# yukara-ikemiya/world-class

Measured on AMD Instinct MI355X. Metric: analysis+synthesis frames/sec (whole node), 48 kHz 5 ms hop, higher is better.
Workload: dtype f64; 1 GPU; 64 synthetic 48 kHz 10 s utterances per GPU (8 distinct, tiled), 5 ms hop, Harvest->CheapTrick->D4C->Synthesis, inputs resident in HBM when the clock starts (`value`; SURVEY.md section 8(d)'s headline with H2D of x and D2H of all outputs inside the clock is `value_with_transfers`); utterances_per_gpu=64, frames_per_gpu=128064, fs=48000, fft_size=2048, parallelism=utterance-sharded x1 (shard.partition), final RCCL all-gather of F0 + checksums

## Files before the change

world_class_amd/csrc/wc_d4c.hip:

```cpp
#include <cmath>
#include <cstdio>
#include <cstdlib>
#include <cstring>
#include <type_traits>
#include <vector>

#include "wc_device.hpp"
#include "wc_internal.hpp"
#include "wc_frames.hpp"
#include "wc_wavefft.hpp"
#include "wc_hostcopy.hpp"

namespace wc {

constexpr double kSafe = 0.000000000001;
constexpr int kMaxBands = 5;

struct D4cArgs {
	const double *x;
	const UttDesc *utts;
	int n_utt;
	const double *tpos, *f0;
	const unsigned long long *rng_off;
	const uint32_t *rng_table;
	unsigned long long rng_base;
	const double2 *tw;
	double *ap;
	double *ap0;
	double *sgd;
	double *coarse;
	uint32_t *cnt;
	const double *nuttall;
	long long total_frames;
	int fs, fft_size_out, n_ap, window_length;
	int select64;
	double threshold;
	long long sgd_stride;
	int *long_list, *long_cnt;
	const int *uidx;
	int rare_only;
	int *rare_list;
};

template <int N, int T>
__device__ __forceinline__ int d4c_windowed(const double *__restrict__ x, int x_len, int fs, double f0, double pos,
											int type, double ratio, const uint32_t *__restrict__ rng,
											unsigned long long roff, double (&wave)[N / T], double *red, int tid) {
	constexpr int EPT = N / T;
	asm volatile("" : "+v"(tid));
	const int hw = mround(ratio * fs / f0 / 2.0);
	const int wl = 2 * hw + 1;
	const int origin = mround(pos * fs + 0.001);
	const double c1 = 2.0 / ratio / fs;
	double cs0, sn0, csd, snd;
	sincospi(f0 * (c1 * (tid - hw)), &sn0, &cs0);
	sincospi(f0 * (c1 * T), &snd, &csd);
	snd = uniform_d(snd);
	csd = uniform_d(csd);
	auto win = [&](double c) { return type == 1 ? fma(0.5, c, 0.5) : fma(c, fma(0.16, c, 0.5), 0.34); };
	double s1 = 0.0, s2 = 0.0;
	{
		double c = cs0, sn = sn0;
#pragma unroll
		for (int e = 0; e < EPT; ++e) {
			const int i = tid + e * T;
			const bool in = i < wl;
			const double w = in ? win(c) : 0.0;
			const int si = clampi(origin + i - hw, 0, x_len - 1);
			const double noise = randn_at(rng, roff + (in ? i : 0)) * kSafe;
			wave[e] = in ? fma(x[si], w, noise) : 0.0;
			s1 += wave[e];
			s2 += w;
			const double cn = fma(c, csd, -(sn * snd));
// ... 57 lines not shown
	if (NONNEG) {
		static_assert(M + 2 >= T + 2 * (T / 64), "P doubles as the scratch of the cumulative sum");
		for (int i = tid; i < len; i += T) S[i] = mir(i) * fs / N;
		__syncthreads();
		seq_cumsum_nonneg<T>(S, len, const_cast<double *>(P), red, tid);
	} else {
		const int ch = (len + T - 1) / T;
		const int lo = tid * ch, hi = min(len, lo + ch);
		double loc = 0.0;
		for (int i = lo; i < hi; ++i) loc += mir(i) * fs / N;
		double run = block_excl_scan<T>(loc, red, tid);
		for (int i = lo; i < hi; ++i) {
			run = mir(i) * fs / N + run;
			S[i] = run;
		}
		__syncthreads();
	}
	const double origin_axis = -(b - 0.5) * fs / N;
	const double step = (double)fs / N, rstep = 1.0 / step;
	auto seg = [&](int i) -> double { return S[min(max(i, 0), len - 1)]; };
	for (int k = tid; k <= M; k += T) {
		double lo_axis = (double)k / N * fs - width / 2.0;
		double hi_axis = lo_axis + width;
		double lo_v = interp1q_rcp(origin_axis, step, rstep, seg, len, lo_axis);
		double hi_v = interp1q_rcp(origin_axis, step, rstep, seg, len, hi_axis);
		out(k, (hi_v - lo_v) / width);
	}
	__syncthreads();
}

__host__ __device__ __forceinline__ bool d4c2_can(double f0, int fs) {
	const int v = (int)(f0 * 4096 / fs);
	return v + 1 <= 120 && v + 2 <= 122;
}

__global__ void d4c_lt_count_kernel(const double *__restrict__ f0, long long total, int fs, uint32_t *__restrict__ cnt,
									const UttDesc *__restrict__ utts, int n_utt, int *__restrict__ uidx, int *__restrict__ long_cnt,
									int *__restrict__ rare_cnt) {
	long long g = (long long)blockIdx.x * blockDim.x + threadIdx.x;
	if (g >= total) return;
	if (g == 0) { *long_cnt = 0; *rare_cnt = 0; }
	uidx[g] = find_utt(utts, n_utt, g);
	double f = f0[g];
	cnt[g] = (f == 0.0) ? 0u : (uint32_t)(2 * mround(3.0 * fs / fmax(f, 40.0) / 2.0) + 1);
}

template <int N, int T>
__global__ __launch_bounds__(T, T == 512 ? 6 : 1) void d4c_lovetrain_kernel(D4cArgs a) {
	constexpr int M = N / 2;
	constexpr int EPT = N / T;
	__shared__ double2 A[fft_lds_size(M)];
	__shared__ double red[2 * (T / 64) + 2];
	double *Ar = reinterpret_cast<double *>(A);
	int tid = threadIdx.x;
	long long g = xcd_frame(blockIdx.x, a.total_frames);
	if (g >= a.total_frames) return;
	const int bins_out = a.fft_size_out / 2 + 1;
	double *__restrict__ row = a.ap + g * (long long)bins_out;
	const double f0v = a.f0[g];
	double ap0 = 0.0;
	if (f0v != 0.0) {
		const int u = find_utt(a.utts, a.n_utt, g);
		const UttDesc ud = a.utts[u];
		const int fs = a.fs;
		const double f0c = fmax(f0v, 40.0);
		double wave[EPT];
// ... 411 lines not shown
		unsigned int acc = inc - own;
		unsigned int d = 4u * lane, cnt;
		if (acc + h4.x >= need) { cnt = h4.x; }
		else if (acc + h4.x + h4.y >= need) { acc += h4.x; d += 1; cnt = h4.y; }
		else if (acc + h4.x + h4.y + h4.z >= need) { acc += h4.x + h4.y; d += 2; cnt = h4.z; }
		else { acc += h4.x + h4.y + h4.z; d += 3; cnt = h4.w; }
		acc = __shfl(acc, first, 64);
		d = __shfl(d, first, 64);
		in_bucket = __shfl(cnt, first, 64);
		need -= acc;
		pre |= ((unsigned long long)d) << shift;
		if (in_bucket == 1u) break;
	}
	double low = 0.0, eq = 0.0, tot = 0.0;
#pragma unroll
	for (int e = 0; e < KEYS; ++e) {
		if (e < nkeys) {
			const double pw = key[e];
			const unsigned long long hb = ((unsigned long long)__double_as_longlong(pw)) >> shift;
			tot += pw;
			low += (hb < (pre >> shift)) ? pw : 0.0;
			eq += (hb == (pre >> shift)) ? pw : 0.0;
		}
	}
	block_sum3<T>(low, eq, tot, red3, tid);
	if (tid == 0) {
		const double thr = (in_bucket == 1u) ? eq : __longlong_as_double((long long)pre);
		const double part = low + (double)need * thr;
		const double cv = 10 * log10(part / tot);
		a.coarse[g * kMaxBands + bnd] = fmin(0.0, cv + (f0 - 100) / 50.0);
	}
}

__global__ __launch_bounds__(256) void d4c_rows_kernel(D4cArgs a) {
	const long long g = blockIdx.x;
	const double f0v = a.f0[g];
	if (f0v == 0.0 || a.ap0[g] <= a.threshold) return;
	const int n_ap = a.n_ap, fs = a.fs;
	const int bins_out = a.fft_size_out / 2 + 1;
	const double *__restrict__ co = a.coarse + g * kMaxBands;
	double *__restrict__ row = a.ap + g * (long long)bins_out;
	const int na = n_ap + 2;
	auto val = [&](int q) { return q == 0 ? -60.0 : (q == na - 1 ? -kSafe : co[q - 1]); };
	for (int k = threadIdx.x; k < bins_out; k += 256) {
		double f = (double)k * fs / a.fft_size_out;
		int c = 1;
		while (c < na && f >= ((c == na - 1) ? fs / 2.0 : c * 3000.0)) ++c;
		c = min(c, na - 1);
		double x0 = (c - 1) * 3000.0;
		double x1 = (c == na - 1) ? fs / 2.0 : c * 3000.0;
		double s = (f - x0) / (x1 - x0);
		double v = val(c - 1) + s * (val(c) - val(c - 1));
		row[k] = exp(v * 0.11512925464970228);
	}
}


constexpr long long kD4Row = 4160;
constexpr int kD4Lds = 2304;

template <int SLOTS>
__device__ __forceinline__ int d4c2_windowed(int type, const double *__restrict__ x, int x_last, int fs, double f0, double pos, double ratio,
											 const uint32_t *__restrict__ rng, int odd, bool weighted, double (&re)[16],
											 double (&im)[16], double &sumsq, int lane) {
	WC_FRESH(lane);
	const int hw = __builtin_amdgcn_readfirstlane(mround(ratio * fs / f0 / 2.0));
	const int wl = 2 * hw + 1;
	const int base = __builtin_amdgcn_readfirstlane(mround(pos * fs + 0.001)) - hw;
	const double c1 = 2.0 / ratio / fs;
	double ce0, se0, co0, so0, cd, sd;
	wf_sincospi(f0 * (c1 * (2 * lane - hw)), se0, ce0);
	wf_sincospi(f0 * (c1 * (2 * lane + 1 - hw)), so0, co0);
	wf_sincospi(f0 * (c1 * 128.0), sd, cd);
	sd = uniform_d(sd);
	cd = uniform_d(cd);
	const double a0 = type == 1 ? 0.5 : 0.34, a2 = type == 1 ? 0.0 : 0.16;
	auto win = [&](double c) { return fma(c, fma(a2, c, 0.5), a0); };
	auto walk = [&](auto loads_c, auto &&body) {
		constexpr int LOADS = decltype(loads_c)::value;
		double ce = ce0, se = se0, co = co0, so = so0;
#pragma unroll
		for (int qg = 0; qg < SLOTS; qg += 4) {
			if (qg * 128 >= wl) break;
			double xs[8];
			uint32_t ns[8];
			const bool ld = LOADS == 1 || (LOADS == 2 && qg >= 16);
			if (ld) {
// ... 108 lines not shown
		ap0 = p1 / p2;
	}
	const bool gate = !(f0v == 0.0 || ap0 <= a.threshold);
	if (lane == 0) {
		a.ap0[g] = ap0;
		a.cnt[g] = gate ? (uint32_t)(3 * (2 * mround(4.0 * a.fs / fmax(47.0, f0v) / 2.0) + 1)) : 0u;
	}
	if (!gate) {
		const double init_val = 1.0 - kSafe;
		for (int k = lane; k < bins_out; k += 64) row[k] = init_val;
	}
}

struct D4Bins {
	double v[2][16];
	double vM;
};
__device__ __forceinline__ void d4c2_dc_correction(D4Bins &s, double f0, int fs, double *L, int lane) {
	constexpr int N = 4096;
	WC_FRESH(lane);
	const int upper = __builtin_amdgcn_readfirstlane(2 + (int)(f0 * N / fs));
	const double dx = -(double)fs / N, rdx = 1.0 / dx;
	L[2 * lane] = s.v[0][0];
	L[2 * lane + 1] = s.v[1][0];
	wf_fence();
	auto rep = [&](int i) {
		const double axis = (double)i * fs / N;
		return interp1q_rcp(f0, dx, rdx, [&](int b) { return L[min(max(b, 0), 127)]; }, upper + 1, axis);
	};
	if (2 * lane < upper - 1) s.v[0][0] += rep(2 * lane);
	if (2 * lane + 1 < upper - 1) s.v[1][0] += rep(2 * lane + 1);
	wf_fence();
}
template <bool NONNEG>
__device__ __forceinline__ void d4c2_smooth(D4Bins &s, double width, int fs, double *L, int lane) {
	constexpr int N = 4096, M = 2048;
	WC_FRESH(lane);
	const int b = __builtin_amdgcn_readfirstlane((int)(width * N / fs) + 1);
	const int len = M + 2 * b + 1;
	int jg[2][4];
#pragma unroll
	for (int p = 0; p < 2; ++p)
#pragma unroll
		for (int gq = 0; gq < 4; ++gq) jg[p][gq] = 2 * wf_j(lane, p, gq) + p;
#pragma unroll
	for (int p = 0; p < 2; ++p)
#pragma unroll
		for (int gq = 0; gq < 4; ++gq)
#pragma unroll
			for (int q = 0; q < 4; ++q) L[jg[p][gq] + 512 * q + b] = s.v[p][4 * gq + q] * fs / N;
	if (lane == 0) L[M + b] = s.vM * fs / N;
	{
		const int ke = 2 * lane, ko = 2 * lane + 1;
		if (ke >= 1 && ke <= b) {
			L[b - ke] = s.v[0][0] * fs / N;
			L[M + b + ke] = s.v[0][7] * fs / N;
		}
		if (ko <= b) {
			L[b - ko] = s.v[1][0] * fs / N;
			L[M + b + ko] = s.v[1][7] * fs / N;
		}
	}
	wf_fence();
	if (NONNEG) {
		seq_cumsum_nonneg_wave<36>(L, len, lane);
	} else {
		seq_cumsum_signed_wave<36>(L, len, lane);
	}
	const double step = (double)fs / N;
	const double origin_axis = -(b - 0.5) * fs / N;
	const double rstep = 1.0 / step;
	const double rwidth = uniform_d(1.0 / width);
	auto at = [&](int k) {
		const double lo_axis = (double)k / N * fs - width / 2.0, hi_axis = lo_axis + width;
		return (wf_interp1q(origin_axis, step, rstep, L, len, hi_axis) - wf_interp1q(origin_axis, step, rstep, L, len, lo_axis)) * rwidth;
	};
#pragma unroll
	for (int p = 0; p < 2; ++p)
#pragma unroll
		for (int gq = 0; gq < 4; ++gq) {
#pragma unroll
			for (int q = 0; q < 4; ++q) s.v[p][4 * gq + q] = at(jg[p][gq] + 512 * q);
			WF_SCHED_FENCE();
		}
	s.vM = at(M);
	wf_fence();
}

#ifndef WC_D4C2_OCC
#define WC_D4C2_OCC 2
#endif
#ifndef WC_D4C2_MASTER_LDS
#define WC_D4C2_MASTER_LDS 1
#endif
#ifndef WC_D4C2_TRACE
#define WC_D4C2_TRACE 0
#endif
#if WC_D4C2_TRACE
#define D4_STAMP(i) do { if (lane == 0) reinterpret_cast<unsigned long long *>(park + 4128)[i] = __builtin_readcyclecounter(); } while (0)
#else
// ... 184 lines not shown
					for (int q = 0; q < 16; ++q) {
						const int i0 = 2 * ln + 128 * q;
						ar[q] *= pw * (i0 + 1.0);
						ai[q] *= pw * (i0 + 2.0);
					}
				}
				wf_r2c4096_half(ar, ai, nyq2, ng, L, a.tw, lane, odd);
#pragma unroll
				for (int s = 0; s < 16; ++s) acc[s] += fma(re[s], ar[s], im[s] * ai[s]);
				accM += nyq1 * nyq2;
				if (odd == 0 && job == 0) D4_STAMP(3);
			}
		}
#pragma unroll
		for (int s = 0; s < 16; ++s) d4_st(row, 1024 * odd + 64 * s + lane, acc[s]);
		if (odd == 0) cenM = accM;
		if (odd == 0) D4_STAMP(4);
	}
	D4_STAMP(5);
	D4Bins cen, sps;
#pragma unroll
	for (int p = 0; p < 2; ++p)
#pragma unroll
		for (int s = 0; s < 16; ++s) {
			cen.v[p][s] = d4_ld(row, 1024 * p + 64 * s + lane);
			sps.v[p][s] = d4_ld(row, 2048 + 1024 * p + 64 * s + lane);
		}
	cen.vM = cenM;
	sps.vM = spsM;
	D4_STAMP(6);
	d4c2_dc_correction(cen, f0, fs, L, lane);
	d4c2_dc_correction(sps, f0, fs, L, lane);
	D4_STAMP(7);
	d4c2_smooth<true>(sps, f0, fs, L, lane);
	D4_STAMP(8);
#pragma unroll
	for (int p = 0; p < 2; ++p)
#pragma unroll
		for (int s = 0; s < 16; ++s) cen.v[p][s] = cen.v[p][s] / sps.v[p][s];
	cen.vM = cen.vM / sps.vM;
#pragma unroll 1
	for (int it = 0; it < 2; ++it) {
		d4c2_smooth<false>(cen, it ? f0 : f0 / 2.0, fs, L, lane);
		if (it == 0) sps = cen;
	}
	D4_STAMP(9);
#pragma unroll
	for (int p = 0; p < 2; ++p)
#pragma unroll
		for (int gq = 0; gq < 4; ++gq) {
			const int j = 2 * wf_j(lane, p, gq) + p;
#pragma unroll
			for (int q = 0; q < 4; ++q) d4_st(row, j + 512 * q, sps.v[p][4 * gq + q] - cen.v[p][4 * gq + q]);
		}
	if (lane == 0) d4_st(row, M, sps.vM - cen.vM);
	D4_STAMP(10);
}

template <bool LONG>
__global__ __launch_bounds__(64) __attribute__((amdgpu_waves_per_eu(WC_D4C2_OCC, WC_D4C2_OCC))) void d4c2_frames_kernel(D4cArgs a) {
	__shared__ __attribute__((aligned(16))) double L[kD4Lds];
	const int lane = threadIdx.x;
	if constexpr (!LONG) {
		const long long g = xcd_frame(blockIdx.x, a.total_frames);
		if (g >= a.total_frames) return;
		d4c2_frame<false>(a, g, L, lane);
	} else {
		const int n_long = *a.long_cnt;
#pragma unroll 1
		for (int i = blockIdx.x; i < n_long; i += gridDim.x) {
			d4c2_frame<true>(a, a.long_list[1 + i], L, lane);
			wf_fence();
		}
	}
}

// ... 7 lines not shown
#define WC_D4C2_BRACKET_FIRST 0x1p-14
#endif
#ifndef WC_D4C2_BAND_PF
#define WC_D4C2_BAND_PF 0
#endif
__global__ __launch_bounds__(64) __attribute__((amdgpu_waves_per_eu(WC_D4C2_BAND_OCC, WC_D4C2_BAND_OCC))) void d4c2_band_kernel(D4cArgs a) {
	constexpr int N = 4096, M = 2048;
	__shared__ __attribute__((aligned(16))) double L[kWfLds];
	const int lane = threadIdx.x;
	const int n_ap = a.n_ap;
	const long long blk = xcd_frame(blockIdx.x, (long long)gridDim.x);
	const long long g = blk / n_ap;
	const int bnd = (int)(blk % n_ap);
	if (g >= a.total_frames) return;
	const double f0v = a.f0[g];
	if (f0v == 0.0 || a.ap0[g] <= a.threshold) return;
	const double f0 = fmax(47.0, f0v);
	const int fs = a.fs;
	const int wln = a.window_length, hwl = wln / 2;
	const int boundary = mround(N * 8.0 / wln);
	const unsigned int K = (unsigned int)(M + 1 - boundary - 1);
	const int center = (int)(3000.0 * (bnd + 1) * N / fs);
	const double *__restrict__ src = a.sgd + g * a.sgd_stride + (center - hwl);
	const int ng = wln > 512 ? 2 : 1;
	double key[2][16], keyM = 0.0;
	[[maybe_unused]] double pf = 0.0;
#pragma unroll
	for (int odd = 0; odd < 2; ++odd) {
		double re[16], im[16], nyq;
		{
			double sv[16], nv[16];
#pragma unroll
			for (int k = 0; k < 16; ++k) {
				const int i = min(2 * lane + 128 * (k >> 1) + (k & 1), wln - 1);
				sv[k] = src[i];
				nv[k] = a.nuttall[i];
			}
#if WC_D4C2_BAND_PF > 0
			if (odd == 0) {
				const long long b2 = min((long long)blockIdx.x + 8ll * WC_D4C2_BAND_PF, (long long)gridDim.x - 1);
				const long long blk2 = xcd_frame(b2, (long long)gridDim.x);
				const long long g2 = min(blk2 / n_ap, a.total_frames - 1);
				const int center2 = (int)(3000.0 * ((int)(blk2 % n_ap) + 1) * N / fs);
				pf = (a.sgd + g2 * a.sgd_stride + (center2 - hwl))[min(16 * lane, wln - 1)];
			}
#endif
			WF_SCHED_FENCE();
#pragma unroll
			for (int q = 0; q < 16; ++q) {
				re[q] = im[q] = 0.0;
				if (q < 8) {
					const int i0 = 2 * lane + 128 * q;
					re[q] = (i0 < wln) ? sv[2 * q] * nv[2 * q] : 0.0;
					im[q] = (i0 + 1 < wln) ? sv[2 * q + 1] * nv[2 * q + 1] : 0.0;
				}
			}
		}
		if (odd) wf_odd_twist(re, im, a.tw, lane, 8);
		if (ng == 1) wdft16<+1, 1>(re, im);
		else wdft16<+1, 2>(re, im);
		wf_fft1024_dit_rest_p<+1>(re, im, L, a.tw, lane, odd);
		if (odd) wf_r2c_unpack_odd(re, im, a.tw, lane);
		else wf_r2c_unpack(re, im, nyq, a.tw, lane);
#pragma unroll
		for (int s = 0; s < 16; ++s) key[odd][s] = fma(re[s], re[s], im[s] * im[s]);
		if (!odd) keyM = nyq * nyq;
	}
	double mx = (lane == 0) ? keyM : 0.0;
#pragma unroll
// ... 65 lines not shown
	for (int p = 0; p < 2; ++p)
#pragma unroll
		for (int s = 0; s < 16; ++s) {
			tot += key[p][s];
			low += (__double_as_longlong(key[p][s]) <= lo) ? key[p][s] : 0.0;
		}
	if (lane == 0) {
		tot += keyM;
		low += (__double_as_longlong(keyM) <= lo) ? keyM : 0.0;
	}
	low = wave_sum_all(low);
	tot = wave_sum_all(tot);
	if (lane == 0) {
		const double part = low + (double)(K - c_lo) * __longlong_as_double(hi);
		const double cv = 10 * log10(part / tot);
		a.coarse[g * kMaxBands + bnd] = fmin(0.0, cv + (f0 - 100) / 50.0);
	}
#if WC_D4C2_BAND_PF > 0
	asm volatile("" ::"v"(pf));
#endif
}


constexpr long long kD4Row1 = 3136;
constexpr int kD4Lds1 = 2176;
__host__ __device__ __forceinline__ bool d4c1_can(double f0, int fs) {
	const int v = (int)(f0 * 2048 / fs);
	return v + 1 <= 120 && v + 2 <= 122;
}
extern "C" int wc_debug_d4c_wave_takes(int fft_size, double f0, int fs) {
	if (fft_size == 4096) return d4c2_can(f0, fs) ? 1 : 0;
	if (fft_size == 2048) return d4c1_can(f0, fs) ? 1 : 0;
	return -1;
}
struct D4Bins1 {
	double v[16];
	double vM;
};
__device__ __forceinline__ void d4c1_dc_correction(D4Bins1 &s, double f0, int fs, double *L, int lane) {
	constexpr int N = 2048;
	WC_FRESH(lane);
	const int upper = __builtin_amdgcn_readfirstlane(2 + (int)(f0 * N / fs));
	const double dx = -(double)fs / N, rdx = 1.0 / dx;
	L[lane] = s.v[0];
	L[64 + lane] = s.v[8];
	wf_fence();
	auto rep = [&](int i) {
		const double axis = (double)i * fs / N;
		return interp1q_rcp(f0, dx, rdx, [&](int b) { return L[min(max(b, 0), 127)]; }, upper + 1, axis);
	};
	if (lane < upper - 1) s.v[0] += rep(lane);
	if (upper - 1 > 64) {
		if (64 + lane < upper - 1) s.v[8] += rep(64 + lane);
	}
	wf_fence();
}
template <bool NONNEG>
__device__ __forceinline__ void d4c1_smooth(D4Bins1 &s, double width, int fs, double *L, int lane) {
	constexpr int N = 2048, M = 1024;
	WC_FRESH(lane);
	const int b = __builtin_amdgcn_readfirstlane((int)(width * N / fs) + 1);
	const int len = M + 2 * b + 1;
	int jg[4];
#pragma unroll
	for (int gq = 0; gq < 4; ++gq) jg[gq] = wf_bin(lane, gq, 0);
#pragma unroll
	for (int gq = 0; gq < 4; ++gq)
#pragma unroll
		for (int q = 0; q < 4; ++q) L[jg[gq] + 256 * q + b] = s.v[4 * gq + q] * fs / N;
	if (lane == 0) L[M + b] = s.vM * fs / N;
	if (lane >= 1 && lane <= b) {
		L[b - lane] = s.v[0] * fs / N;
		L[M + b + lane] = s.v[7] * fs / N;
	}
	if (64 + lane <= b) {
		L[b - 64 - lane] = s.v[8] * fs / N;
		L[M + b + 64 + lane] = s.v[15] * fs / N;
	}
	wf_fence();
	if (NONNEG) seq_cumsum_nonneg_wave<20>(L, len, lane);
	else seq_cumsum_signed_wave<20>(L, len, lane);
	const double step = (double)fs / N;
	const double origin_axis = -(b - 0.5) * fs / N;
	const double rstep = 1.0 / step;
	const double rwidth = uniform_d(1.0 / width);
	auto at = [&](int k) {
		const double lo_axis = (double)k / N * fs - width / 2.0, hi_axis = lo_axis + width;
		return (wf_interp1q(origin_axis, step, rstep, L, len, hi_axis) - wf_interp1q(origin_axis, step, rstep, L, len, lo_axis)) * rwidth;
	};
#pragma unroll
	for (int gq = 0; gq < 4; ++gq) {
#pragma unroll
		for (int q = 0; q < 4; ++q) s.v[4 * gq + q] = at(jg[gq] + 256 * q);
		WF_SCHED_FENCE();
	}
	s.vM = at(M);
	wf_fence();
}

#ifndef WC_D4C1_LT_OCC
#define WC_D4C1_LT_OCC 3
#endif
#ifndef WC_D4C1_OCC
#define WC_D4C1_OCC 2
#endif
#ifndef WC_D4C1_BAND_OCC
#define WC_D4C1_BAND_OCC 3
#endif
__global__ __launch_bounds__(64) __attribute__((amdgpu_waves_per_eu(WC_D4C1_LT_OCC, WC_D4C1_LT_OCC))) void d4c1_lovetrain_kernel(D4cArgs a) {
	constexpr int N = 2048, M = 1024;
	__shared__ __attribute__((aligned(16))) double L[kWfLds];
	const int lane = threadIdx.x;
	const long long g = xcd_frame(blockIdx.x, a.total_frames);
	if (g >= a.total_frames) return;
	const int bins_out = a.fft_size_out / 2 + 1;
	double *__restrict__ row = a.ap + g * (long long)bins_out;
	const double f0v = a.f0[g];
	const int fs = a.fs;
	const double f0c = uniform_d(fmax(f0v, 40.0));
	double ap0 = 0.0;
	if (f0v != 0.0) {
		const int u = a.uidx[g];
		const UttDesc ud = a.utts[u];
		const int b0 = (int)ceil(100.0 * N / fs);
		const int b1 = (int)ceil(4000.0 * N / fs);
		const int b2 = min((int)ceil(7900.0 * N / fs), M);
		double p1 = 0.0, p2 = 0.0;
		double re[16], im[16], unused, nyq;
		const int wl = d4c2_windowed<16>(2, a.x + ud.x_off, ud.x_len - 1, fs, f0c, a.tpos[g], 3.0, a.rng_table + (a.rng_off[g] - a.rng_base), 0,
// ... 98 lines not shown
				for (int q = 0; q < 16; ++q) {
					const int i0 = 2 * l2 + 128 * q;
					ar[q] *= i0 + 1.0;
					ai[q] *= i0 + 2.0;
				}
			}
			wf_r2c4096_half(ar, ai, nyq2, ng, L, a.tw, ln, 0);
			double acc[16];
#pragma unroll
			for (int s = 0; s < 16; ++s) acc[s] = fma(re[s], ar[s], im[s] * ai[s]);
			if (job == 1) {
				double prev[16];
#pragma unroll
				for (int s = 0; s < 16; ++s) prev[s] = d4_ld(row, 64 * s + ln);
				WF_SCHED_FENCE();
#pragma unroll
				for (int s = 0; s < 16; ++s) acc[s] += prev[s];
			}
#pragma unroll
			for (int s = 0; s < 16; ++s) d4_st(row, 64 * s + ln, acc[s]);
			cenM += nyq1 * nyq2;
		}
	}
	D4Bins1 cen, sps;
#pragma unroll
	for (int s = 0; s < 16; ++s) {
		cen.v[s] = d4_ld(row, 64 * s + lane);
		sps.v[s] = d4_ld(row, 1024 + 64 * s + lane);
	}
	cen.vM = cenM;
	sps.vM = spsM;
	d4c1_dc_correction(cen, f0, fs, L, lane);
	d4c1_dc_correction(sps, f0, fs, L, lane);
	d4c1_smooth<true>(sps, f0, fs, L, lane);
#pragma unroll
	for (int s = 0; s < 16; ++s) cen.v[s] = cen.v[s] / sps.v[s];
	cen.vM = cen.vM / sps.vM;
#pragma unroll 1
	for (int it = 0; it < 2; ++it) {
		d4c1_smooth<false>(cen, it ? f0 : f0 / 2.0, fs, L, lane);
		if (it == 0) sps = cen;
	}
#pragma unroll
	for (int gq = 0; gq < 4; ++gq) {
		const int j = wf_bin(lane, gq, 0);
#pragma unroll
		for (int q = 0; q < 4; ++q) d4_st(row, j + 256 * q, sps.v[4 * gq + q] - cen.v[4 * gq + q]);
	}
	if (lane == 0) d4_st(row, M, sps.vM - cen.vM);
}

__global__ __launch_bounds__(64) __attribute__((amdgpu_waves_per_eu(WC_D4C1_BAND_OCC, WC_D4C1_BAND_OCC))) void d4c1_band_kernel(D4cArgs a) {
	constexpr int N = 2048, M = 1024;
	__shared__ __attribute__((aligned(16))) double L[kWfLds];
	const int lane = threadIdx.x;
	const int n_ap = a.n_ap;
	const long long blk = xcd_frame(blockIdx.x, (long long)gridDim.x);
	const long long g = blk / n_ap;
	const int bnd = (int)(blk % n_ap);
	if (g >= a.total_frames) return;
	const double f0v = a.f0[g];
	if (f0v == 0.0 || a.ap0[g] <= a.threshold) return;
	const double f0 = fmax(47.0, f0v);
	const int fs = a.fs;
	const int wln = a.window_length, hwl = wln / 2;
	const int boundary = mround(N * 8.0 / wln);
	const unsigned int K = (unsigned int)(M + 1 - boundary - 1);
	const int center = (int)(3000.0 * (bnd + 1) * N / fs);
	const double *__restrict__ src = a.sgd + g * a.sgd_stride + (center - hwl);
	const int ng = wln > 512 ? 2 : 1;
	double key[16], keyM = 0.0;
	{
		double re[16], im[16], nyq;
		{
			double sv[16], nv[16];
#pragma unroll
			for (int k = 0; k < 16; ++k) {
				const int i = min(2 * lane + 128 * (k >> 1) + (k & 1), wln - 1);
				sv[k] = src[i];
				nv[k] = a.nuttall[i];
			}
			WF_SCHED_FENCE();
#pragma unroll
			for (int q = 0; q < 16; ++q) {
				re[q] = im[q] = 0.0;
				if (q < 8) {
					const int i0 = 2 * lane + 128 * q;
					re[q] = (i0 < wln) ? sv[2 * q] * nv[2 * q] : 0.0;
					im[q] = (i0 + 1 < wln) ? sv[2 * q + 1] * nv[2 * q + 1] : 0.0;
				}
			}
		}
		wf_r2c4096_half(re, im, nyq, ng, L, a.tw, lane, 0);
#pragma unroll
		for (int s = 0; s < 16; ++s) key[s] = fma(re[s], re[s], im[s] * im[s]);
		keyM = nyq * nyq;
	}
	double mx = (lane == 0) ? keyM : 0.0;
#pragma unroll
	for (int s = 0; s < 16; ++s) mx = fmax(mx, key[s]);
#pragma unroll
	for (int o = 32; o > 0; o >>= 1) mx = fmax(mx, __shfl_down(mx, o, 64));
	mx = uniform_d(mx);
	long long lo = -1, hi = __double_as_longlong(mx);
	unsigned int c_lo = 0;
	auto count_le = [&](long long t) {
		unsigned int c = (unsigned int)__popcll(__ballot(lane == 0 && __double_as_longlong(keyM) <= t));
#pragma unroll
		for (int s = 0; s < 16; ++s) c += (unsigned int)__popcll(__ballot(__double_as_longlong(key[s]) <= t));
		return c;
	};
	if (!a.select64) {
		auto count_hi = [&](int h) {
// ... 32 lines not shown
		const long long mid = lo + ((hi - lo) >> 1);
		const unsigned int c = count_le(mid);
		if (c >= K) hi = mid;
		if (c <= K) { lo = mid; c_lo = c; }
		if (c == K) break;
	}
	double low = 0.0, tot = 0.0;
#pragma unroll
	for (int s = 0; s < 16; ++s) {
		tot += key[s];
		low += (__double_as_longlong(key[s]) <= lo) ? key[s] : 0.0;
	}
	if (lane == 0) {
		tot += keyM;
		low += (__double_as_longlong(keyM) <= lo) ? keyM : 0.0;
	}
	low = wave_sum_all(low);
	tot = wave_sum_all(tot);
	if (lane == 0) {
		const double part = low + (double)(K - c_lo) * __longlong_as_double(hi);
		const double cv = 10 * log10(part / tot);
		a.coarse[g * kMaxBands + bnd] = fmin(0.0, cv + (f0 - 100) / 50.0);
	}
}

}

using namespace wc;

struct wc_d4c {
	int fs, fft_size_d4c, fft_size_lt, n_ap, window_length;
	double threshold;
	bool select64 = false;
	bool split;
	bool wave2;
	Device *dev;
	double f0_bound = 0.0;
	DevBuf nuttall, utts, cnt, uidx, long_list, rare_list, off, endpos, endpos2, ap0, sgd, coarse, d_x, d_tpos, d_f0, d_ap;
	HostBuf h_stage, h_rows, h_x;
};

template <int N>
static void launch_lt(const D4cArgs &a, hipStream_t s) {
	long long blocks = ((a.total_frames + 7) / 8) * 8;
	constexpr int TL = (N >= 8192) ? 1024 : (N / 8 < 64 ? 64 : N / 8);
	hipLaunchKernelGGL((d4c_lovetrain_kernel<N, TL>), dim3((unsigned)blocks), dim3(TL), 0, s, a);
}
template <int N>
static void launch_main(const D4cArgs &a, hipStream_t s, bool split, int part) {
	long long blocks = ((a.total_frames + 7) / 8) * 8;
	constexpr int TF = (N >= 8192) ? 1024 : (N / 8 < 64 ? 64 : N / 8);
	if (part == 0) {
		if (!split) hipLaunchKernelGGL((d4c_frames_kernel<N, TF, false>), dim3((unsigned)blocks), dim3(TF), 0, s, a);
		else hipLaunchKernelGGL((d4c_frames_kernel<N, TF, true>), dim3((unsigned)blocks), dim3(TF), 0, s, a);
		return;
	}
	if (a.n_ap > 0) hipLaunchKernelGGL((d4c_band_kernel<N, TF>), dim3((unsigned)(blocks * a.n_ap)), dim3(TF), 0, s, a);
	hipLaunchKernelGGL(d4c_rows_kernel, dim3((unsigned)a.total_frames), dim3(256), 0, s, a);
}

int d4c_enqueue(wc_d4c *d, hipStream_t s, int n_utt, const double *d_x, const int *x_length, const double *d_tpos,
				const double *d_f0, const int *f0_length, int fft_size, double *d_ap, const uint64_t *rng_pos,
				const unsigned long long *d_start) {
	Device *dev = d->dev;
	if (fft_size < 2 || (fft_size & 1)) return fail(WC_ERR_INVALID, "d4c: fft_size must be even and positive");
	std::vector<UttDesc> utts(n_utt);
	long long xo = 0, fo = 0;
	uint64_t min_pos = ~0ull, max_end = 0;
	const uint64_t lt_max = (uint64_t)(2 * (int)(3.0 * d->fs / 40.0 / 2.0 + 1.0) + 1);
	const uint64_t main_max = 3ull * (uint64_t)(2 * (int)(4.0 * d->fs / 47.0 / 2.0 + 1.0) + 1);
	for (int u = 0; u < n_utt; ++u) {
		if (x_length[u] <= 0 || f0_length[u] < 0) return fail(WC_ERR_INVALID, "d4c: non-positive length");
		UttDesc &t = utts[u];
		t.x_off = xo; t.f_off = fo; t.y_off = 0;
		t.x_len = x_length[u]; t.f_len = f0_length[u]; t.y_len = 0; t.f_base = 0;
		t.rng_pos = rng_pos ? rng_pos[u] : 0ull;
		xo += x_length[u];
		fo += f0_length[u];
		if (t.rng_pos < min_pos) min_pos = t.rng_pos;
		uint64_t e = t.rng_pos + (lt_max + main_max) * (uint64_t)t.f_len;
		if (e > max_end) max_end = e;
	}
	const long long total = fo;
	(void)min_pos; (void)max_end;
	if (total == 0) return WC_OK;
	int rc;
	if ((rc = d->utts.reserve(sizeof(UttDesc) * n_utt))) return rc;
	if ((rc = d->cnt.reserve(sizeof(uint32_t) * total))) return rc;
	if ((rc = d->uidx.reserve(sizeof(int) * total))) return rc;
	if ((rc = d->long_list.reserve(sizeof(int) * (total + 1)))) return rc;
	if ((rc = d->rare_list.reserve(sizeof(int) * (total + 1)))) return rc;
	if ((rc = d->off.reserve(sizeof(uint64_t) * total))) return rc;
	if ((rc = d->ap0.reserve(sizeof(double) * total))) return rc;
	const bool split = d->split;
	const bool main2 = d->wave2 && split && (d->fft_size_d4c == 4096 || d->fft_size_d4c == 2048) && d->window_length <= 1023;
	const long long row2 = d->fft_size_d4c == 4096 ? kD4Row : kD4Row1;
	if (split) {
		if ((rc = d->sgd.reserve(sizeof(double) * (size_t)total * (main2 ? (size_t)row2 : (size_t)(d->fft_size_d4c / 2 + 1))))) return rc;
		if ((rc = d->coarse.reserve(sizeof(double) * (size_t)total * kMaxBands))) return rc;
	}
	if ((rc = d->endpos.reserve(sizeof(uint64_t) * n_utt))) return rc;
	if ((rc = d->endpos2.reserve(sizeof(uint64_t) * n_utt))) return rc;
	if ((rc = d->h_stage.reserve(sizeof(UttDesc) * n_utt + sizeof(uint64_t) * n_utt))) return rc;
	std::memcpy(d->h_stage.p, utts.data(), sizeof(UttDesc) * n_utt);
	WC_HIP(hipMemcpyAsync(d->utts.p, d->h_stage.p, sizeof(UttDesc) * n_utt, hipMemcpyHostToDevice, s));
	if ((rc = d->h_stage.mark(s))) return rc;
	const unsigned grid1 = (unsigned)((total + 255) / 256);
	hipLaunchKernelGGL(d4c_lt_count_kernel, dim3(grid1), dim3(256), 0, s, d_f0, total, d->fs, d->cnt.as<uint32_t>(), d->utts.as<UttDesc>(), n_utt,
					   d->uidx.as<int>(), d->long_list.as<int>(), d->rare_list.as<int>());
	hipLaunchKernelGGL(utt_scan_kernel, dim3(n_utt), dim3(256), 0, s, d->cnt.as<uint32_t>(), d->utts.as<UttDesc>(),
					   d_start, d->off.as<unsigned long long>(), d->endpos.as<unsigned long long>());
	D4cArgs a;
	a.x = d_x; a.utts = d->utts.as<UttDesc>(); a.n_utt = n_utt; a.tpos = d_tpos; a.f0 = d_f0;
	a.rng_off = d->off.as<unsigned long long>(); a.rng_table = dev->rng_table.as<uint32_t>(); a.rng_base = dev->rng_base;
	a.tw = dev->twiddle; a.ap = d_ap; a.ap0 = d->ap0.as<double>(); a.cnt = d->cnt.as<uint32_t>(); a.uidx = d->uidx.as<int>(); a.long_cnt = d->long_list.as<int>(); a.long_list = d->long_list.as<int>();
	a.sgd = d->sgd.as<double>(); a.coarse = d->coarse.as<double>();
	a.nuttall = d->nuttall.as<double>(); a.total_frames = total; a.fs = d->fs; a.fft_size_out = fft_size;
	a.n_ap = d->n_ap; a.window_length = d->window_length; a.threshold = d->threshold; a.select64 = d->select64 ? 1 : 0;
	a.rare_only = 0;
	a.rare_list = d->rare_list.as<int>();
	a.sgd_stride = main2 ? row2 : (long long)(d->fft_size_d4c / 2 + 1);
	const long long blocks8 = ((total + 7) / 8) * 8;
	if ((rc = dev->time_begin("d4c_lovetrain", s))) return rc;
	if (d->wave2 && d->fft_size_lt == 4096) {
		hipLaunchKernelGGL(d4c2_lovetrain_kernel<false>, dim3((unsigned)blocks8), dim3(64), 0, s, a);
		hipLaunchKernelGGL(d4c2_lovetrain_kernel<true>, dim3((unsigned)blocks8), dim3(64), 0, s, a);
	} else if (d->wave2 && d->fft_size_lt == 2048) {
		hipLaunchKernelGGL(d4c1_lovetrain_kernel, dim3((unsigned)blocks8), dim3(64), 0, s, a);
	}
	else switch (d->fft_size_lt) {
		case 1024: launch_lt<1024>(a, s); break;
		case 2048: launch_lt<2048>(a, s); break;
		case 4096: launch_lt<4096>(a, s); break;
		case 8192: launch_lt<8192>(a, s); break;
		default: return fail(WC_ERR_UNSUPPORTED, "d4c: unsupported LoveTrain FFT size (fs must be 8..96 kHz)");
	}
	WC_HIP(hipGetLastError());
	if ((rc = dev->time_end("d4c_lovetrain", s))) return rc;
	hipLaunchKernelGGL(utt_scan_kernel, dim3(n_utt), dim3(256), 0, s, d->cnt.as<uint32_t>(), d->utts.as<UttDesc>(),
					   d->endpos.as<unsigned long long>(), d->off.as<unsigned long long>(), d->endpos2.as<unsigned long long>());
	for (int part = 0; part < (split ? 2 : 1); ++part) {
		const char *name = part == 0 ? "d4c_frames" : "d4c_bands";
		if ((rc = dev->time_begin(name, s))) return rc;
		if (main2 && part == 0) {
			a.rare_only = 1;
			if (d->fft_size_d4c == 4096) {
				hipLaunchKernelGGL(d4c2_frames_kernel<false>, dim3((unsigned)blocks8), dim3(64), 0, s, a);
				hipLaunchKernelGGL(d4c2_frames_kernel<true>, dim3((unsigned)std::min<long long>(blocks8, 4096)), dim3(64), 0, s, a);
				hipLaunchKernelGGL((d4c_frames_kernel<4096, 512, true, true>), dim3(256), dim3(512), 0, s, a);
			} else {
				hipLaunchKernelGGL(d4c1_frames_kernel, dim3((unsigned)blocks8), dim3(64), 0, s, a);
				hipLaunchKernelGGL((d4c_frames_kernel<2048, 256, true, true>), dim3(256), dim3(256), 0, s, a);
			}
			a.rare_only = 0;
		} else if (main2 && part == 1) {
			if (a.n_ap > 0) {
				if (d->fft_size_d4c == 4096) hipLaunchKernelGGL(d4c2_band_kernel, dim3((unsigned)(blocks8 * a.n_ap)), dim3(64), 0, s, a);
				else hipLaunchKernelGGL(d4c1_band_kernel, dim3((unsigned)(blocks8 * a.n_ap)), dim3(64), 0, s, a);
			}
			hipLaunchKernelGGL(d4c_rows_kernel, dim3((unsigned)a.total_frames), dim3(256), 0, s, a);
		} else
		switch (d->fft_size_d4c) {
			case 1024: launch_main<1024>(a, s, split, part); break;
			case 2048: launch_main<2048>(a, s, split, part); break;
			case 4096: launch_main<4096>(a, s, split, part); break;
			case 8192: launch_main<8192>(a, s, split, part); break;
			default: return fail(WC_ERR_UNSUPPORTED, "d4c: unsupported FFT size (fs must be 8..96 kHz)");
		}
		WC_HIP(hipGetLastError());
		if ((rc = dev->time_end(name, s))) return rc;
	}
#if WC_D4C2_TRACE
	if (const char *path = getenv("WC_D4C_TRACE")) {
		std::vector<double> row((size_t)kD4Row);
		std::vector<unsigned long long> out;
		WC_HIP(hipStreamSynchronize(s));
		for (long long g = 0; g < total; g += 7) {
			WC_HIP(hipMemcpy(row.data(), d->sgd.as<double>() + g * kD4Row, sizeof(double) * kD4Row, hipMemcpyDeviceToHost));
			const unsigned long long *st = reinterpret_cast<const unsigned long long *>(row.data() + 4128);
			out.insert(out.end(), st, st + 16);
		}
		if (FILE *f = fopen(path, "wb")) { fwrite(out.data(), 8, out.size(), f); fclose(f); }
	}
#endif
	return WC_OK;
}

void d4c_set_f0_bound(wc_d4c *d, double f0_bound) { d->f0_bound = f0_bound; }
const unsigned long long *d4c_end_positions(const wc_d4c *d) { return d->endpos2.as<unsigned long long>(); }

uint64_t d4c_draw_bound(const wc_d4c *d, int f0_length) {
	const uint64_t lt_max = (uint64_t)(2 * (int)(3.0 * d->fs / 40.0 / 2.0 + 1.0) + 1);
	const uint64_t main_max = 3ull * (uint64_t)(2 * (int)(4.0 * d->fs / 47.0 / 2.0 + 1.0) + 1);
// ... 12 lines not shown
		lo = p0 < lo ? p0 : lo;
		uint64_t e = p0 + d4c_draw_bound(d, f0_length[u]);
		hi = e > hi ? e : hi;
		total += f0_length[u] > 0 ? f0_length[u] : 0;
	}
	if ((rc = dev->ensure_rng(lo, hi))) return rc;
	if ((rc = d4c_enqueue(d, s, n_utt, d_x, x_length, d_tpos, d_f0, f0_length, fft_size, d_ap, rng_pos, nullptr))) return rc;
	if (rng_pos && total > 0) {
		std::vector<uint64_t> h_end(n_utt);
		WC_HIP(hipMemcpyAsync(h_end.data(), d->endpos2.p, sizeof(uint64_t) * n_utt, hipMemcpyDeviceToHost, s));
		WC_HIP(hipStreamSynchronize(s));
		for (int u = 0; u < n_utt; ++u) rng_pos[u] = h_end[u];
	}
	return WC_OK;
}

wc::Device *d4c_device(const wc_d4c *d) { return d->dev; }

extern "C" {

wc_d4c *wc_d4c_create(int fs, double threshold) {
	if (fs <= 0) { set_error("d4c: fs must be positive"); return nullptr; }
	Device *dev = current_device();
	if (!dev) return nullptr;
	wc_d4c *d = new wc_d4c();
	d->fs = fs;
	d->threshold = threshold;
	d->dev = dev;
	{
		const char *sp = getenv("WC_D4C_SPLIT");
		d->split = !(sp && sp[0] == '0');
		const char *sel = getenv("WC_D4C_SELECT");
		d->select64 = sel && std::strcmp(sel, "64") == 0;
		const char *impl = getenv("WC_D4C_IMPL");
		d->wave2 = !(impl && std::strcmp(impl, "block") == 0);
	}
	d->fft_size_d4c = static_cast<int>(std::pow(2.0, 1.0 + static_cast<int>(std::log(4.0 * fs / 47.0 + 1) / 0.69314718055994529)));
	d->n_ap = static_cast<int>(std::fmin(15000.0, fs / 2.0 - 3000.0) / 3000.0);
	d->window_length = static_cast<int>(3000.0 * d->fft_size_d4c / fs) * 2 + 1;
	d->fft_size_lt = static_cast<int>(std::pow(2.0, 1.0 + static_cast<int>(std::log(3.0 * fs / 40.0 + 1) / 0.69314718055994529)));
	if (d->n_ap < 0) d->n_ap = 0;
	if (d->n_ap > kMaxBands || (d->fft_size_d4c != 1024 && d->fft_size_d4c != 2048 && d->fft_size_d4c != 4096 && d->fft_size_d4c != 8192) ||
		(d->fft_size_lt != 1024 && d->fft_size_lt != 2048 && d->fft_size_lt != 4096 && d->fft_size_lt != 8192)) {
		set_error("d4c: unsupported sampling rate (supported: 8 kHz .. 96 kHz)");
		delete d;
		return nullptr;
	}
	std::vector<double> win(d->window_length);
	for (int i = 0; i < d->window_length; ++i) {
		double t = i / (d->window_length - 1.0);
		win[i] = 0.355768 - 0.487396 * std::cos(2.0 * 3.1415926535897932384 * t) +
				 0.144232 * std::cos(4.0 * 3.1415926535897932384 * t) - 0.012604 * std::cos(6.0 * 3.1415926535897932384 * t);
	}
	if (d->nuttall.reserve(sizeof(double) * win.size()) ||
		hipMemcpy(d->nuttall.p, win.data(), sizeof(double) * win.size(), hipMemcpyHostToDevice) != hipSuccess) {
		set_error("d4c: window upload failed");
		delete d;
		return nullptr;
	}
	dev->handle_born();
	return d;
}
void wc_d4c_destroy(wc_d4c *d) {
	if (!d) return;
	d->dev->quiesce();
	d->dev->handle_gone();
// ... 43 lines not shown
```

Before: 5.195 million frames/s.

## Truncate D4C spectral smoothing to bins consumed by bands; batch rows kernel over frames

Adds a tail rule that computes, per frame, how many spectral bins the downstream band aperiodicity stage actually reads, then shortens the cumulative-sum smoothing passes and skips divides and stores beyond that bin range, using smaller cumsum templates when the length allows. The band kernels now skip loading window samples past the window length. The per-frame rows kernel is reorganised so each block covers a 256-bin chunk across 8 frames, computing the interpolation segment once per bin. An environment switch restores full-length smoothing. The risk is subtle numerical changes if the computed bound misjudges which bins are needed.

```diff
diff --git a/world_class_amd/csrc/wc_d4c.hip b/world_class_amd/csrc/wc_d4c.hip
--- a/world_class_amd/csrc/wc_d4c.hip
+++ b/world_class_amd/csrc/wc_d4c.hip
@@ -39,6 +39,7 @@
 	int *long_list, *long_cnt;
 	const int *uidx;
 	int rare_only;
+	int tail_full;
 	int *rare_list;
 };
 
@@ -162,6 +163,33 @@
 __host__ __device__ __forceinline__ bool d4c2_can(double f0, int fs) {
 	const int v = (int)(f0 * 4096 / fs);
 	return v + 1 <= 120 && v + 2 <= 122;
+}
+
+struct D4Tail {
+	int len[3], last[3];
+};
+__host__ __device__ __forceinline__ D4Tail d4c_tail_rule(int N, int fs, int n_ap, int window_length, double f0) {
+	const int M = N / 2;
+	D4Tail t;
+	int need = n_ap > 0 ? (int)(3000.0 * n_ap * N / fs) + window_length / 2 : M;
+#pragma unroll
+	for (int i = 2; i >= 0; --i) {
+		const double width = i == 1 ? f0 / 2.0 : f0;
+		const int b = (int)(width * N / fs) + 1;
+		int len = need + b + (int)(width * N / fs / 2.0) + 3;
+		if (need >= M || len > M + b) {
+			len = M + 2 * b + 1;
+			need = need >= M ? M : need;
+		}
+		t.last[i] = need < M ? need : M;
+		t.len[i] = len;
+		need = len - 1 - b < M ? len - 1 - b : M;
+	}
+	return t;
+}
+__host__ __device__ __forceinline__ int d4c_tail_bound(int N, int len) {
+	const int ch = (len + 63) / 64;
+	return N == 4096 ? (ch <= 28 ? 28 : 36) : (ch <= 14 ? 14 : 20);
 }
 
 __global__ void d4c_lt_count_kernel(const double *__restrict__ f0, long long total, int fs, uint32_t *__restrict__ cnt,
@@ -639,27 +667,42 @@
 	}
 }
 
+constexpr int kD4RowsFrames = 8;
 __global__ __launch_bounds__(256) void d4c_rows_kernel(D4cArgs a) {
-	const long long g = blockIdx.x;
-	const double f0v = a.f0[g];
-	if (f0v == 0.0 || a.ap0[g] <= a.threshold) return;
 	const int n_ap = a.n_ap, fs = a.fs;
 	const int bins_out = a.fft_size_out / 2 + 1;
-	const double *__restrict__ co = a.coarse + g * kMaxBands;
-	double *__restrict__ row = a.ap + g * (long long)bins_out;
+	const unsigned chunks = (unsigned)(bins_out + 255) / 256u;
+	const int k = (int)(blockIdx.x % chunks) * 256 + threadIdx.x;
+	const long long g0 = (long long)(blockIdx.x / chunks) * kD4RowsFrames;
+	bool gate[kD4RowsFrames];
+#pragma unroll
+	for (int i = 0; i < kD4RowsFrames; ++i) {
+		const long long g = min(g0 + i, a.total_frames - 1);
+		gate[i] = g0 + i < a.total_frames && !(a.f0[g] == 0.0 || a.ap0[g] <= a.threshold);
+	}
+	if (k >= bins_out) return;
 	const int na = n_ap + 2;
-	auto val = [&](int q) { return q == 0 ? -60.0 : (q == na - 1 ? -kSafe : co[q - 1]); };
-	for (int k = threadIdx.x; k < bins_out; k += 256) {
-		double f = (double)k * fs / a.fft_size_out;
-		int c = 1;
-		while (c < na && f >= ((c == na - 1) ? fs / 2.0 : c * 3000.0)) ++c;
-		c = min(c, na - 1);
-		double x0 = (c - 1) * 3000.0;
-		double x1 = (c == na - 1) ? fs / 2.0 : c * 3000.0;
-		double s = (f - x0) / (x1 - x0);
+	double f = (double)k * fs / a.fft_size_out;
+	int c = 1;
+	while (c < na && f >= ((c == na - 1) ? fs / 2.0 : c * 3000.0)) ++c;
+	c = min(c, na - 1);
+	double x0 = (c - 1) * 3000.0;
+	double x1 = (c == na - 1) ? fs / 2.0 : c * 3000.0;
+	const double s = (f - x0) / (x1 - x0);
+#pragma unroll
+	for (int i = 0; i < kD4RowsFrames; ++i) {
+		if (!gate[i]) continue;
+		const long long g = g0 + i;
+		const double *__restrict__ co = a.coarse + g * kMaxBands;
+		auto val = [&](int q) { return q == 0 ? -60.0 : (q == na - 1 ? -kSafe : co[q - 1]); };
 		double v = val(c - 1) + s * (val(c) - val(c - 1));
-		row[k] = exp(v * 0.11512925464970228);
-	}
+		a.ap[g * (long long)bins_out + k] = exp(v * 0.11512925464970228);
+	}
+}
+static void launch_rows(const D4cArgs &a, hipStream_t s) {
+	const int bins_out = a.fft_size_out / 2 + 1;
+	const long long blocks = (long long)((bins_out + 255) / 256) * ((a.total_frames + kD4RowsFrames - 1) / kD4RowsFrames);
+	hipLaunchKernelGGL(d4c_rows_kernel, dim3((unsigned)blocks), dim3(256), 0, s, a);
 }
 
 
@@ -834,12 +877,14 @@
 	if (2 * lane + 1 < upper - 1) s.v[1][0] += rep(2 * lane + 1);
 	wf_fence();
 }
+__host__ __device__ constexpr int d4c2_slot_first(int p, int g, int q) {
+	return 2 * ((g == 0 ? 0 : g == 1 ? (p ? 192 : 128) : g == 2 ? 64 : (p ? 128 : 129)) + 256 * q) + p;
+}
 template <bool NONNEG>
-__device__ __forceinline__ void d4c2_smooth(D4Bins &s, double width, int fs, double *L, int lane) {
+__device__ __forceinline__ void d4c2_smooth(D4Bins &s, double width, int fs, double *L, int lane, int len) {
 	constexpr int N = 4096, M = 2048;
 	WC_FRESH(lane);
 	const int b = __builtin_amdgcn_readfirstlane((int)(width * N / fs) + 1);
-	const int len = M + 2 * b + 1;
 	int jg[2][4];
 #pragma unroll
 	for (int p = 0; p < 2; ++p)
@@ -854,20 +899,24 @@
 	if (lane == 0) L[M + b] = s.vM * fs / N;
 	{
 		const int ke = 2 * lane, ko = 2 * lane + 1;
+		const bool high = len > M + b;
 		if (ke >= 1 && ke <= b) {
 			L[b - ke] = s.v[0][0] * fs / N;
-			L[M + b + ke] = s.v[0][7] * fs / N;
+			if (high) L[M + b + ke] = s.v[0][7] * fs / N;
 		}
 		if (ko <= b) {
 			L[b - ko] = s.v[1][0] * fs / N;
-			L[M + b + ko] = s.v[1][7] * fs / N;
+			if (high) L[M + b + ko] = s.v[1][7] * fs / N;
 		}
 	}
 	wf_fence();
+	const bool small = d4c_tail_bound(N, len) == 28;
 	if (NONNEG) {
-		seq_cumsum_nonneg_wave<36>(L, len, lane);
+		if (small) seq_cumsum_nonneg_wave<28>(L, len, lane);
+		else seq_cumsum_nonneg_wave<36>(L, len, lane);
 	} else {
-		seq_cumsum_signed_wave<36>(L, len, lane);
+		if (small) seq_cumsum_signed_wave<28>(L, len, lane);
+		else seq_cumsum_signed_wave<36>(L, len, lane);
 	}
 	const double step = (double)fs / N;
 	const double origin_axis = -(b - 0.5) * fs / N;
@@ -1118,16 +1167,35 @@
 	d4c2_dc_correction(cen, f0, fs, L, lane);
 	d4c2_dc_correction(sps, f0, fs, L, lane);
 	D4_STAMP(7);
-	d4c2_smooth<true>(sps, f0, fs, L, lane);
+	int tl_len[3], tl_last[3];
+	auto rule = [&]() {
+		const D4Tail t = d4c_tail_rule(4096, fs, a.tail_full ? 0 : a.n_ap, a.window_length, f0);
+#pragma unroll
+		for (int i = 0; i < 3; ++i) {
+			tl_len[i] = __builtin_amdgcn_readfirstlane(t.len[i]);
+			tl_last[i] = __builtin_amdgcn_readfirstlane(t.last[i]);
+		}
+	};
+	if constexpr (!LONG) rule();
+	auto tail = [&](int stage, int &len, int &last) {
+		if constexpr (LONG) rule();
+		len = stage == 0 ? tl_len[0] : stage == 1 ? tl_len[1] : tl_len[2];
+		last = stage == 0 ? tl_last[0] : stage == 1 ? tl_last[1] : tl_last[2];
+	};
+	int t_len, t_last;
+	tail(0, t_len, t_last);
+	d4c2_smooth<true>(sps, f0, fs, L, lane, t_len);
 	D4_STAMP(8);
 #pragma unroll
 	for (int p = 0; p < 2; ++p)
 #pragma unroll
-		for (int s = 0; s < 16; ++s) cen.v[p][s] = cen.v[p][s] / sps.v[p][s];
-	cen.vM = cen.vM / sps.vM;
+		for (int s = 0; s < 16; ++s)
+			if ((s & 3) < 3 || d4c2_slot_first(p, s >> 2, s & 3) <= t_last) cen.v[p][s] = cen.v[p][s] / sps.v[p][s];
+	if (t_last >= M) cen.vM = cen.vM / sps.vM;
 #pragma unroll 1
 	for (int it = 0; it < 2; ++it) {
-		d4c2_smooth<false>(cen, it ? f0 : f0 / 2.0, fs, L, lane);
+		tail(1 + it, t_len, t_last);
+		d4c2_smooth<false>(cen, it ? f0 : f0 / 2.0, fs, L, lane, t_len);
 		if (it == 0) sps = cen;
 	}
 	D4_STAMP(9);
@@ -1201,9 +1269,12 @@
 			double sv[16], nv[16];
 #pragma unroll
 			for (int k = 0; k < 16; ++k) {
-				const int i = min(2 * lane + 128 * (k >> 1) + (k & 1), wln - 1);
-				sv[k] = src[i];
-				nv[k] = a.nuttall[i];
+				sv[k] = nv[k] = 0.0;
+				if (128 * (k >> 1) < wln) {
+					const int i = min(2 * lane + 128 * (k >> 1) + (k & 1), wln - 1);
+					sv[k] = src[i];
+					nv[k] = a.nuttall[i];
+				}
 			}
 #if WC_D4C2_BAND_PF > 0
 			if (odd == 0) {
@@ -1335,6 +1406,17 @@
 	if (fft_size == 4096) return d4c2_can(f0, fs) ? 1 : 0;
 	if (fft_size == 2048) return d4c1_can(f0, fs) ? 1 : 0;
 	return -1;
+}
+extern "C" int wc_debug_d4c_read_bins(int fft_size, int fs, int n_ap, int window_length, double f0, int *out) {
+	if (fft_size != 4096 && fft_size != 2048) return -1;
+	const D4Tail t = d4c_tail_rule(fft_size, fs, n_ap, window_length, f0);
+	for (int i = 0; i < 3; ++i) {
+		out[i] = t.len[i];
+		out[3 + i] = t.last[i];
+		out[6 + i] = d4c_tail_bound(fft_size, t.len[i]);
+	}
+	out[9] = n_ap > 0 ? (int)(3000.0 * n_ap * fft_size / fs) + window_length / 2 : fft_size / 2;
+	return 0;
 }
 struct D4Bins1 {
 	double v[16];
@@ -1358,12 +1440,12 @@
 	}
 	wf_fence();
 }
+__host__ __device__ constexpr int d4c1_slot_first(int g, int q) { return (g == 0 ? 0 : g == 1 ? 128 : g == 2 ? 64 : 129) + 256 * q; }
 template <bool NONNEG>
-__device__ __forceinline__ void d4c1_smooth(D4Bins1 &s, double width, int fs, double *L, int lane) {
+__device__ __forceinline__ void d4c1_smooth(D4Bins1 &s, double width, int fs, double *L, int lane, int len, int last) {
 	constexpr int N = 2048, M = 1024;
 	WC_FRESH(lane);
 	const int b = __builtin_amdgcn_readfirstlane((int)(width * N / fs) + 1);
-	const int len = M + 2 * b + 1;
 	int jg[4];
 #pragma unroll
 	for (int gq = 0; gq < 4; ++gq) jg[gq] = wf_bin(lane, gq, 0);
@@ -1372,17 +1454,24 @@
 #pragma unroll
 		for (int q = 0; q < 4; ++q) L[jg[gq] + 256 * q + b] = s.v[4 * gq + q] * fs / N;
 	if (lane == 0) L[M + b] = s.vM * fs / N;
+	const bool high = len > M + b;
 	if (lane >= 1 && lane <= b) {
 		L[b - lane] = s.v[0] * fs / N;
-		L[M + b + lane] = s.v[7] * fs / N;
+		if (high) L[M + b + lane] = s.v[7] * fs / N;
 	}
 	if (64 + lane <= b) {
 		L[b - 64 - lane] = s.v[8] * fs / N;
-		L[M + b + 64 + lane] = s.v[15] * fs / N;
+		if (high) L[M + b + 64 + lane] = s.v[15] * fs / N;
 	}
 	wf_fence();
-	if (NONNEG) seq_cumsum_nonneg_wave<20>(L, len, lane);
-	else seq_cumsum_signed_wave<20>(L, len, lane);
+	const bool small = d4c_tail_bound(N, len) == 14;
+	if (NONNEG) {
+		if (small) seq_cumsum_nonneg_wave<14>(L, len, lane);
+		else seq_cumsum_nonneg_wave<20>(L, len, lane);
+	} else {
+		if (small) seq_cumsum_signed_wave<14>(L, len, lane);
+		else seq_cumsum_signed_wave<20>(L, len, lane);
+	}
 	const double step = (double)fs / N;
 	const double origin_axis = -(b - 0.5) * fs / N;
 	const double rstep = 1.0 / step;
@@ -1394,10 +1483,13 @@
 #pragma unroll
 	for (int gq = 0; gq < 4; ++gq) {
 #pragma unroll
-		for (int q = 0; q < 4; ++q) s.v[4 * gq + q] = at(jg[gq] + 256 * q);
+		for (int q = 0; q < 4; ++q) {
+			if (q < 3 || d4c1_slot_first(gq, q) <= last) s.v[4 * gq + q] = at(jg[gq] + 256 * q);
+			else s.v[4 * gq + q] = 0.0;
+		}
 		WF_SCHED_FENCE();
 	}
-	s.vM = at(M);
+	s.vM = last >= M ? at(M) : 0.0;
 	wf_fence();
 }
 
@@ -1562,22 +1654,40 @@
 	sps.vM = spsM;
 	d4c1_dc_correction(cen, f0, fs, L, lane);
 	d4c1_dc_correction(sps, f0, fs, L, lane);
-	d4c1_smooth<true>(sps, f0, fs, L, lane);
-#pragma unroll
-	for (int s = 0; s < 16; ++s) cen.v[s] = cen.v[s] / sps.v[s];
-	cen.vM = cen.vM / sps.vM;
+	int tl_len[3], tl_last[3];
+	{
+		const D4Tail t = d4c_tail_rule(2048, fs, a.tail_full ? 0 : a.n_ap, a.window_length, f0);
+#pragma unroll
+		for (int i = 0; i < 3; ++i) {
+			tl_len[i] = __builtin_amdgcn_readfirstlane(t.len[i]);
+			tl_last[i] = __builtin_amdgcn_readfirstlane(t.last[i]);
+		}
+	}
+	auto tail = [&](int stage, int &len, int &last) {
+		len = stage == 0 ? tl_len[0] : stage == 1 ? tl_len[1] : tl_len[2];
+		last = stage == 0 ? tl_last[0] : stage == 1 ? tl_last[1] : tl_last[2];
+	};
+	int t_len, t_last;
+	tail(0, t_len, t_last);
+	d4c1_smooth<true>(sps, f0, fs, L, lane, t_len, t_last);
+#pragma unroll
+	for (int s = 0; s < 16; ++s)
+		if ((s & 3) < 3 || d4c1_slot_first(s >> 2, s & 3) <= t_last) cen.v[s] = cen.v[s] / sps.v[s];
+	if (t_last >= M) cen.vM = cen.vM / sps.vM;
 #pragma unroll 1
 	for (int it = 0; it < 2; ++it) {
-		d4c1_smooth<false>(cen, it ? f0 : f0 / 2.0, fs, L, lane);
+		tail(1 + it, t_len, t_last);
+		d4c1_smooth<false>(cen, it ? f0 : f0 / 2.0, fs, L, lane, t_len, t_last);
 		if (it == 0) sps = cen;
 	}
 #pragma unroll
 	for (int gq = 0; gq < 4; ++gq) {
 		const int j = wf_bin(lane, gq, 0);
 #pragma unroll
-		for (int q = 0; q < 4; ++q) d4_st(row, j + 256 * q, sps.v[4 * gq + q] - cen.v[4 * gq + q]);
-	}
-	if (lane == 0) d4_st(row, M, sps.vM - cen.vM);
+		for (int q = 0; q < 4; ++q)
+			if (q < 3 || d4c1_slot_first(gq, q) <= t_last) d4_st(row, j + 256 * q, sps.v[4 * gq + q] - cen.v[4 * gq + q]);
+	}
+	if (lane == 0 && t_last >= M) d4_st(row, M, sps.vM - cen.vM);
 }
 
 __global__ __launch_bounds__(64) __attribute__((amdgpu_waves_per_eu(WC_D4C1_BAND_OCC, WC_D4C1_BAND_OCC))) void d4c1_band_kernel(D4cArgs a) {
@@ -1606,9 +1716,12 @@
 			double sv[16], nv[16];
 #pragma unroll
 			for (int k = 0; k < 16; ++k) {
-				const int i = min(2 * lane + 128 * (k >> 1) + (k & 1), wln - 1);
-				sv[k] = src[i];
-				nv[k] = a.nuttall[i];
+				sv[k] = nv[k] = 0.0;
+				if (128 * (k >> 1) < wln) {
+					const int i = min(2 * lane + 128 * (k >> 1) + (k & 1), wln - 1);
+					sv[k] = src[i];
+					nv[k] = a.nuttall[i];
+				}
 			}
 			WF_SCHED_FENCE();
 #pragma unroll
@@ -1707,6 +1820,7 @@
 	int fs, fft_size_d4c, fft_size_lt, n_ap, window_length;
 	double threshold;
 	bool select64 = false;
+	bool tail_full = false;
 	bool split;
 	bool wave2;
 	Device *dev;
@@ -1731,7 +1845,7 @@
 		return;
 	}
 	if (a.n_ap > 0) hipLaunchKernelGGL((d4c_band_kernel<N, TF>), dim3((unsigned)(blocks * a.n_ap)), dim3(TF), 0, s, a);
-	hipLaunchKernelGGL(d4c_rows_kernel, dim3((unsigned)a.total_frames), dim3(256), 0, s, a);
+	launch_rows(a, s);
 }
 
 int d4c_enqueue(wc_d4c *d, hipStream_t s, int n_utt, const double *d_x, const int *x_length, const double *d_tpos,
@@ -1793,6 +1907,7 @@
 	a.nuttall = d->nuttall.as<double>(); a.total_frames = total; a.fs = d->fs; a.fft_size_out = fft_size;
 	a.n_ap = d->n_ap; a.window_length = d->window_length; a.threshold = d->threshold; a.select64 = d->select64 ? 1 : 0;
 	a.rare_only = 0;
+	a.tail_full = d->tail_full ? 1 : 0;
 	a.rare_list = d->rare_list.as<int>();
 	a.sgd_stride = main2 ? row2 : (long long)(d->fft_size_d4c / 2 + 1);
 	const long long blocks8 = ((total + 7) / 8) * 8;
@@ -1833,7 +1948,7 @@
 				if (d->fft_size_d4c == 4096) hipLaunchKernelGGL(d4c2_band_kernel, dim3((unsigned)(blocks8 * a.n_ap)), dim3(64), 0, s, a);
 				else hipLaunchKernelGGL(d4c1_band_kernel, dim3((unsigned)(blocks8 * a.n_ap)), dim3(64), 0, s, a);
 			}
-			hipLaunchKernelGGL(d4c_rows_kernel, dim3((unsigned)a.total_frames), dim3(256), 0, s, a);
+			launch_rows(a, s);
 		} else
 		switch (d->fft_size_d4c) {
 			case 1024: launch_main<1024>(a, s, split, part); break;
@@ -1912,6 +2027,8 @@
 		d->split = !(sp && sp[0] == '0');
 		const char *sel = getenv("WC_D4C_SELECT");
 		d->select64 = sel && std::strcmp(sel, "64") == 0;
+		const char *tail = getenv("WC_D4C_TAIL");
+		d->tail_full = tail && std::strcmp(tail, "full") == 0;
 		const char *impl = getenv("WC_D4C_IMPL");
 		d->wave2 = !(impl && std::strcmp(impl, "block") == 0);
 	}
```

After: 5.234 million frames/s (median of 6 runs). About the same (+0.7%).
